# HI-ComputerVision/uni-encoder-code

Measured on AMD Instinct MI355X. Metric: img/s fwd+bwd Swin-L 1024x2048 bs=2 per GPU, higher is better.
Workload: dtype bf16; 1 GPU; BASELINE configs[2]: full OneFormer (Swin-L ws12 backbone + MSDeformAttn pixel decoder + 150-query masked-attention decoder), 1024x2048, fwd+bwd, synthetic loss; global_batch=2, parallelism=dp1, mode=eval() (train_mode reported separately with --full)

## Files before the change

include/uenc.h:

```cpp
#ifndef UENC_H
#define UENC_H
#include <stdint.h>

#ifdef __cplusplus
extern "C" {
#endif

#define UENC_F32 0
#define UENC_BF16 1

#ifndef UENC_STREAM_T
#define UENC_STREAM_T void*
#endif
typedef UENC_STREAM_T uenc_stream_t;

#define UENC_EPI_NONE 0
#define UENC_EPI_GELU 1
#define UENC_EPI_RELU 2
#define UENC_EPI_RESIDUAL 3
#define UENC_EPI_MUL_DGELU 4
#define UENC_EPI_MUL_DRELU 5

int uenc_version(void);
const char* uenc_arch(void);

int uenc_cast_f32_bf16(const float* src, void* dst, long n , uenc_stream_t stream);
int uenc_dropout_bf16(const void* in, void* out, long n, unsigned seed, float p, uenc_stream_t stream);
int uenc_cast_transpose_f32_bf16(const float* src , void* dst , int R, int C, uenc_stream_t stream);

int uenc_cast_multi(const void* table, int n, long total_tiles, uenc_stream_t stream);

int uenc_upsample_bilinear(const float* in, float* out, long NC, int Hi, int Wi, int Ho, int Wo, uenc_stream_t stream);

int uenc_attn_mask(const float* logits, uint8_t* mask, long rows, int Hi, int Wi, int Ho, int Wo, uenc_stream_t stream);

int uenc_add_cast_bf16(const float* a, const float* b, void* out, long n, long period, uenc_stream_t stream);
int uenc_msda_prep_fwd(const float* offaw, long ld, const float* ref, int ref_per_image, const int64_t* shapes, float* loc,
                       float* aw, long rows, int Lq, int M, int L, int P, uenc_stream_t stream);
int uenc_msda_prep_bwd(const float* dloc, const float* daw, const float* aw, const int64_t* shapes, void* doffaw, long ld,
                       long rows, int Lq, int M, int L, int P, uenc_stream_t stream);
int uenc_segment_colsum(const void* x16, long ld, int cols, const int64_t* seg_start, int nseg, long rows_per_image, int images,
                        float* out, uenc_stream_t stream);

long uenc_groupnorm_tokens_scratch_bytes(int B, int HW, int C, int G);
int uenc_groupnorm_tokens_fwd(const void* x, int x_dtype, const float* gamma, const float* beta, void* y, int y_dtype,
                              float* stats, void* scratch, const float* add_src, int Hs, int Ws, int H, int W, int B, int HW,
                              int C, int G, float eps, int relu, uenc_stream_t stream);
int uenc_groupnorm_tokens_bwd(const void* dy, int dy_dtype, const void* x, int x_dtype, const float* gamma, const float* beta,
                              const float* stats, void* dx, int dx_dtype, float* dgamma, float* dbeta, void* scratch, int B,
                              int HW, int C, int G, int relu, uenc_stream_t stream);
int uenc_upsample_bilinear_tokens_bwd(const void* dy, int dy_dtype, float* dsrc, int B, int H, int W, int Hs, int Ws, int C,
                                      uenc_stream_t stream);
int uenc_merge_nearest_tokens_fwd(const void* a, int a_dtype, const void* prev, int prev_dtype, void* out, int out_dtype, int B, int H, int W,
                                  int Hs, int Ws, int C, uenc_stream_t stream);
int uenc_merge_nearest_tokens_bwd(const void* dy, int dy_dtype, float* dprev, int B, int H, int W, int Hs, int Ws, int C,
                                  uenc_stream_t stream);
int uenc_im2col3x3(const void* in, void* col, int B, int H, int W, int C, uenc_stream_t stream);
int uenc_col2im3x3(const void* dcol, void* dx, int B, int H, int W, int C, uenc_stream_t stream);
int uenc_im2col3x3_s2(const void* in, void* col, int B, int H, int W, int C, uenc_stream_t stream);
int uenc_col2im3x3_s2(const void* dcol, float* dx, int B, int H, int W, int C, uenc_stream_t stream);

int uenc_gemm_nt(const void* A, int a_dtype, long lda, const void* W, long ldw, void* C, int c_dtype, long ldc,
                 int M, int N, int K, const float* bias, int epilogue, const void* aux, long ldaux,
                 void* aux_out, long ldaux_out, float alpha, int splitk, int accumulate, uenc_stream_t stream);
#define UENC_NT_TILE_256X256 256
#define UENC_NT_TILE_256X192 192
#define UENC_NT_TILE_128X256 128
int uenc_gemm_nt_tile(const void* A, int a_dtype, long lda, const void* W, long ldw, void* C, int c_dtype, long ldc,
                      int M, int N, int K, const float* bias, int epilogue, const void* aux, long ldaux,
                      void* aux_out, long ldaux_out, float alpha, int splitk, int accumulate, int tile, uenc_stream_t stream);
int uenc_gemm_nt_scaled(const void* A, int a_dtype, long lda, const void* W, long ldw, void* C, int c_dtype, long ldc,
                        int M, int N, int K, const float* bias, int epilogue, const void* aux, long ldaux,
                        void* aux_out, long ldaux_out, float alpha, const float* sample_scale, int rows_per_sample, uenc_stream_t stream);
int uenc_gemm_nt_ln(const void* A, int a_dtype, long lda, const void* W, long ldw, void* C, long ldc, int M, int N, int K, const float* bias,
                    const void* residual, long ldres, const float* gamma, const float* beta, float eps, float* y32, void* y16, float* stats,
                    uenc_stream_t stream);
int uenc_gemm_nt_splits(int K, int splitk);
int uenc_gemm_nt_partials(const void* A, int a_dtype, long lda, const void* W, long ldw, float* P, long ldp, long part_stride,
                          int M, int N, int K, float alpha, int splitk, uenc_stream_t stream);

int uenc_gemm_nt_batched(const void* A, int a_dtype, long lda, long bsA, const void* W, long ldw, long bsW, void* C, int c_dtype,
                         long ldc, long bsC, int batch, int M, int N, int K, float alpha, int splitk, int accumulate, uenc_stream_t stream);

int uenc_gemm_tn(const void* dY, int dy_dtype, long ldy, const void* X, int x_dtype, long ldx, float* dW, long ldw,
                 float* db, int M, int N, int K, int splitm, uenc_stream_t stream);
int uenc_gemm_tn_tile(const void* dY, int dy_dtype, long ldy, const void* X, int x_dtype, long ldx, float* dW, long ldw,
                      float* db, int M, int N, int K, int splitm, int tile, uenc_stream_t stream);
int uenc_gemm_tn_scaled(const void* dY, int dy_dtype, long ldy, const void* X, int x_dtype, long ldx, float* dW, long ldw,
                        float* db, int M, int N, int K, int splitm, float alpha, uenc_stream_t stream);

int uenc_gemm_tn_grouped(const void* table, int n, int total_items, int tile, double flops, uenc_stream_t stream);
int uenc_gemm_tn_grouped_small(const void* table, int n, int total_items, double flops, uenc_stream_t stream);

int uenc_layernorm_fwd(const void* x, int x_dtype, const void* res, int res_dtype, float* h_out, const float* gamma,
                       const float* beta, void* y, int y_dtype, float* stats, long M, int C, float eps, void* y16,
                       uenc_stream_t stream);
int uenc_layernorm_bwd(const void* dy, int dy_dtype, const void* h, int h_dtype, const float* stats, const float* gamma,
                       const float* dres, void* dx, int dx_dtype, float* dgamma, float* dbeta, long M, int C, void* dx16,
                       float* part_ws, int defer_param_sums, uenc_stream_t stream);
int uenc_layernorm_bwd_blocks(long M, int C);
int uenc_ln_param_grouped(const void* table, int n, int total_groups, uenc_stream_t stream);
int uenc_patch_merge_ln_fwd(const float* x, const float* gamma, const float* beta, void* y, float* stats, int B, int H, int W,
                            int C, float eps, uenc_stream_t stream);
int uenc_patch_merge_ln_bwd(const void* dy, int dy_dtype, const float* x, const float* stats, const float* gamma, float* dx,
                            float* dgamma, float* dbeta, float* part_ws, int B, int H, int W, int C, int defer_param_sums,
                            uenc_stream_t stream);

int uenc_window_attn_np(int ws);
int uenc_relpos_expand(const float* table , float* bias_q ,
                       float* bias_k , int nH, int ws, uenc_stream_t stream);
int uenc_relpos_expand_grouped(const void* table, int n, int total_blocks, uenc_stream_t stream);
int uenc_window_attn_fwd(const void* qkv, const void* qkv_bias, const float* bias_q, void* out, float* lse, int B, int H, int W,
                         int C, int nH, int ws, int shift, float scale, uenc_stream_t stream);
long uenc_window_attn_bwd_ws_floats(int B, int H, int W, int nH, int ws);
int uenc_window_attn_bwd(const void* qkv, const void* qkv_bias, const float* bias_q, const float* bias_k,
                         const void* o_saved, const float* lse , const void* d_out, void* dqkv,
                         float* dS_ws, float* dtable, float* dbias_pad,
                         int B, int H, int W, int C, int nH, int ws, int shift, float scale, int defer_dtable, uenc_stream_t stream);
int uenc_window_attn_bwd_groups(int B, int H, int W, int nH, int ws);
int uenc_window_attn_dtable_grouped(const void* table, int n, int total_blocks, uenc_stream_t stream);

int uenc_msdeform_attn_fwd(const void* value, int v_dtype, const int64_t* shapes, const int64_t* level_start,
                           const float* loc, const float* attn, void* out, int out_dtype, int B, int S, int M, int D,
                           int L, int Lq, int P, uenc_stream_t stream);
int uenc_msdeform_attn_fwd_tiled(const void* value, int v_dtype, const int64_t* shapes, const int64_t* level_start,
                                 const float* loc, const float* attn, void* out, int out_dtype, int B, int S, int M, int D,
                                 int L, int Lq, int P, const int64_t* shapes_host, uenc_stream_t stream);
int uenc_msdeform_attn_bwd(const void* value, int v_dtype, const int64_t* shapes, const int64_t* level_start,
                           const float* loc, const float* attn, const void* grad_out, int go_dtype, float* grad_value,
                           float* grad_loc, float* grad_attn, int B, int S, int M, int D, int L, int Lq, int P,
                           const int64_t* shapes_host, void* workspace, long workspace_bytes, uenc_stream_t stream);
long uenc_msdeform_attn_bwd_workspace_bytes(const int64_t* shapes_host, int B, int M, int D, int L, int Lq, int P);
int uenc_msdeform_attn_fused_fwd(const void* value, int v_dtype, const int64_t* shapes, const int64_t* level_start, const float* offaw,
                                 long ld, const float* ref, int ref_per_image, void* out, int out_dtype, int B, int S, int M, int D,
                                 int L, int Lq, int P, uenc_stream_t stream);
int uenc_msdeform_attn_fused_fwd_tiled(const void* value, int v_dtype, const int64_t* shapes, const int64_t* level_start, const float* offaw,
                                       long ld, const float* ref, int ref_per_image, void* out, int out_dtype, int B, int S, int M, int D,
                                       int L, int Lq, int P, const int64_t* shapes_host, uenc_stream_t stream);
int uenc_msdeform_attn_fused_bwd(const void* value, int v_dtype, const int64_t* shapes, const int64_t* level_start, const float* offaw,
                                 long ld, const float* ref, int ref_per_image, const void* grad_out, int go_dtype, float* grad_value,
                                 void* doffaw, long ld_doffaw, int B, int S, int M, int D, int L, int Lq, int P, const int64_t* shapes_host,
                                 void* workspace, long workspace_bytes, uenc_stream_t stream);

long uenc_mha_fwd_workspace_floats(int B, int H, int Lq, int S);
int uenc_mha_fwd(const void* q, long q_bs, long q_rs, const void* k, long k_bs, long k_rs, const void* v, long v_bs,
                 long v_rs, const unsigned char* mask, long mask_rs, void* out, long o_bs, long o_rs, float* lse,
                 float* workspace, int B, int H, int Lq, int S, float scale, float dropout_p, unsigned seed, uenc_stream_t stream);
int uenc_mha_bwd(const void* q, long q_bs, long q_rs, const void* k, long k_bs, long k_rs, const void* v, long v_bs,
                 long v_rs, const unsigned char* mask, long mask_rs, const void* out, long o_bs, long o_rs,
                 const float* lse, const void* dout, long do_bs, long do_rs, float* dq, long dq_bs, long dq_rs, void* dk,
                 long dk_bs, long dk_rs, void* dv, long dv_bs, long dv_rs, int B, int H, int Lq, int S, float scale,
                 float dropout_p, unsigned seed, uenc_stream_t stream);

int uenc_na2d_fwd(const void* qkv, const float* rpb, void* out, float* lse, int B, int H, int W, int nH, int K, int dilation,
                  float scale, uenc_stream_t stream);
int uenc_na2d_bwd(const void* qkv, const float* rpb, const void* out, const void* dout, const float* lse, void* dqkv, float* drpb,
                  float* delta_ws, int B, int H, int W, int nH, int K, int dilation, float scale, uenc_stream_t stream);

int uenc_postproc_semantic(const float* mask_logits, const float* class_prob, float* sem, int Q, int C, int Cp, int hl, int wl,
                           int Hp, int Wp, int Ho, int Wo, uenc_stream_t stream);
int uenc_postproc_panoptic_stats(const float* mask_logits, const float* score, int* ids, int* counts, int Q, int hl, int wl, int Hp,
                                 int Wp, int Ho, int Wo, uenc_stream_t stream);
int uenc_postproc_panoptic_label(const float* mask_logits, const int* ids, const int* segid, int* seg, int Q, int hl, int wl, int Hp,
                                 int Wp, int Ho, int Wo, uenc_stream_t stream);

int uenc_gemm_nt_f32(const float* A, long lda, const float* W, long ldw, float* C, long ldc, int M, int N, int K, const float* bias,
                     int epilogue, const float* aux, long ldaux, float* aux_out, long ldaux_out, float alpha, int accumulate, uenc_stream_t stream);
int uenc_gemm_tn_f32(const float* dY, long ldy, const float* X, long ldx, float* dW, long ldw, float* db, int M, int N, int K, uenc_stream_t stream);
int uenc_window_attn_f32_fwd(const float* qkv, const float* qkv_bias, const float* table, float* out, int B, int H, int W, int C, int nH,
                             int ws, int shift, float scale, uenc_stream_t stream);
int uenc_window_attn_f32_bwd(const float* qkv, const float* qkv_bias, const float* table, const float* dout, float* dqkv, float* dtable,
                             float* dbias_pad, int B, int H, int W, int C, int nH, int ws, int shift, float scale, uenc_stream_t stream);
int uenc_mha_f32_fwd(const float* q, long qs0, long qs1, const float* k, long ks0, long ks1, const float* v, long vs0, long vs1,
                     const uint8_t* mask, long mask_row_stride, float* out, long os0, long os1, float* lse, int B, int nH, int Lq, int S,
                     float scale, float dropout_p, unsigned seed, uenc_stream_t stream);
int uenc_mha_f32_bwd(const float* q, long qs0, long qs1, const float* k, long ks0, long ks1, const float* v, long vs0, long vs1,
                     const uint8_t* mask, long mask_row_stride, const float* out, long os0, long os1, const float* lse, const float* dout,
                     long gos0, long gos1, float* dq, long dqs0, long dqs1, float* dk, long dks0, long dks1, float* dv, long dvs0, long dvs1,
                     float* delta, int B, int nH, int Lq, int S, float scale, float dropout_p, unsigned seed, uenc_stream_t stream);
int uenc_na2d_f32_fwd(const float* qkv, const float* rpb, float* out, float* lse, int B, int H, int W, int nH, int K, int dilation,
                      float scale, uenc_stream_t stream);
int uenc_na2d_f32_bwd(const float* qkv, const float* rpb, const float* out, const float* dout, const float* lse, float* dqkv, float* drpb,
                      int B, int H, int W, int nH, int K, int dilation, float scale, uenc_stream_t stream);
// ... 104 lines not shown
```

uni-encoder-code_amd/csrc/layernorm.hip:

```cpp
#include "common.h"
#include <stdlib.h>

struct LnFwd {
    const void* x; int x_f32;
    const void* res; int res_f32;
    float* h_out;
    const float* gamma; const float* beta;
    void* y; int y_f32;
    bf16* y16;
    float2* stats;
    long M; int C; float eps;
    int mgH, mgW, mgC;
};

struct PatchGather {
    long base; bool ok[4];
    __device__ __forceinline__ PatchGather(long row, int H, int W, int C) {
        const int W2 = (W + 1) >> 1, H2 = (H + 1) >> 1;
        const int j = (int)(row % W2);
        const long r2 = row / W2;
        const int i = (int)(r2 % H2);
        const long b = r2 / H2;
        base = ((b * H + 2 * i) * W + 2 * j) * C;
        const bool y1 = 2 * i + 1 < H, x1 = 2 * j + 1 < W;
        ok[0] = true; ok[1] = y1; ok[2] = x1; ok[3] = y1 && x1;
    }
};
__device__ __forceinline__ void patch_col(int c, int W, int C, int& seg, long& off) {
    seg = c / C;
    off = ((long)(seg & 1) * W + (seg >> 1)) * C + (c - seg * C);
}

__device__ __forceinline__ float4 load4(const void* base, int is_f32, long idx) {
    if (is_f32) return *(const float4*)((const float*)base + idx);
    const bf16x4 v = *(const bf16x4*)((const bf16*)base + idx);
    return make_float4((float)v[0], (float)v[1], (float)v[2], (float)v[3]);
}
__device__ __forceinline__ void store4(void* base, int is_f32, long idx, float4 v) {
    if (is_f32) { *(float4*)((float*)base + idx) = v; return; }
    bf16x4 o; o[0] = (bf16)v.x; o[1] = (bf16)v.y; o[2] = (bf16)v.z; o[3] = (bf16)v.w;
    *(bf16x4*)((bf16*)base + idx) = o;
}

template <int NV, bool MG>
__global__ __launch_bounds__(256) void ln_fwd_kernel(LnFwd p) {
    const int lane = threadIdx.x & 63;
    const long wave0 = (long)blockIdx.x * 4 + (threadIdx.x >> 6);
    const long nwaves = (long)gridDim.x * 4;
    const float invC = 1.0f / (float)p.C;
    int gseg[NV];
    long goff[NV];
    if (MG) {
#pragma unroll
        for (int i = 0; i < NV; ++i) patch_col(min(lane * 4 + i * 256, p.C - 4), p.mgW, p.mgC, gseg[i], goff[i]);
    }
    for (long row = wave0; row < p.M; row += nwaves) {
        float4 v[NV];
        float s = 0.f;
        const PatchGather pg(MG ? row : 0, MG ? p.mgH : 1, MG ? p.mgW : 1, p.mgC);
#pragma unroll
        for (int i = 0; i < NV; ++i) {
            const int c = lane * 4 + i * 256;
            if (c < p.C) {
                if (MG) v[i] = pg.ok[gseg[i]] ? *(const float4*)((const float*)p.x + pg.base + goff[i]) : make_float4(0.f, 0.f, 0.f, 0.f);
                else v[i] = load4(p.x, p.x_f32, row * p.C + c);
                if (p.res != nullptr) {
                    const float4 r = load4(p.res, p.res_f32, row * p.C + c);
                    v[i].x += r.x; v[i].y += r.y; v[i].z += r.z; v[i].w += r.w;
                }
                if (p.h_out != nullptr) *(float4*)(p.h_out + row * p.C + c) = v[i];
                s += v[i].x + v[i].y + v[i].z + v[i].w;
            } else {
                v[i] = make_float4(0.f, 0.f, 0.f, 0.f);
            }
        }
        const float mean = wave_sum(s) * invC;
        float q = 0.f;
#pragma unroll
        for (int i = 0; i < NV; ++i) {
            const int c = lane * 4 + i * 256;
            if (c < p.C) {
                const float a = v[i].x - mean, b = v[i].y - mean, cc = v[i].z - mean, d = v[i].w - mean;
                q += a * a + b * b + cc * cc + d * d;
            }
        }
        const float rstd = rsqrtf(wave_sum(q) * invC + p.eps);
        if (p.stats != nullptr && lane == 0) p.stats[row] = make_float2(mean, rstd);
#pragma unroll
        for (int i = 0; i < NV; ++i) {
            const int c = lane * 4 + i * 256;
            if (c < p.C) {
                const float4 g = *(const float4*)(p.gamma + c), b = *(const float4*)(p.beta + c);
                float4 o;
                o.x = (v[i].x - mean) * rstd * g.x + b.x;
                o.y = (v[i].y - mean) * rstd * g.y + b.y;
                o.z = (v[i].z - mean) * rstd * g.z + b.z;
                o.w = (v[i].w - mean) * rstd * g.w + b.w;
                store4(p.y, p.y_f32, row * p.C + c, o);
                if (p.y16 != nullptr) store4(p.y16, 0, row * p.C + c, o);
            }
        }
    }
}

#define LN_LAUNCH(DIR, NVV, GRID, BLOCK, SHM, STREAM, P)                                                          \
    do {                                                                                                          \
        if ((P).mgC > 0) hipLaunchKernelGGL((ln_##DIR##_kernel<NVV, true>), GRID, BLOCK, SHM, STREAM, P);        \
        else hipLaunchKernelGGL((ln_##DIR##_kernel<NVV, false>), GRID, BLOCK, SHM, STREAM, P);                   \
    } while (0)

static int ln_fwd_launch(LnFwd& p, hipStream_t stream);

extern "C" int uenc_layernorm_fwd(const void* x, int x_dtype, const void* res, int res_dtype, float* h_out,
                                  const float* gamma, const float* beta, void* y, int y_dtype, float* stats,
                                  long M, int C, float eps, void* y16, hipStream_t stream) {
    UENC_CHECK_ARG(x && gamma && beta && y && M > 0 && C > 0 && C % 4 == 0 && C <= 6144);
    LnFwd p;
    p.x = x; p.x_f32 = (x_dtype == UENC_F32); p.res = res; p.res_f32 = (res_dtype == UENC_F32);
    p.h_out = h_out; p.gamma = gamma; p.beta = beta; p.y = y; p.y_f32 = (y_dtype == UENC_F32); p.y16 = (bf16*)y16;
    p.stats = (float2*)stats; p.M = M; p.C = C; p.eps = eps; p.mgH = p.mgW = p.mgC = 0;
    return ln_fwd_launch(p, stream);
}

static int ln_fwd_launch(LnFwd& p, hipStream_t stream) {
// ... 50 lines not shown
        const float2 st = p.stats[row];
        float4 d[NV], xh[NV], rs[NV];
        float s1 = 0.f, s2 = 0.f;
        const PatchGather pg(MG ? row : 0, MG ? p.mgH : 1, MG ? p.mgW : 1, p.mgC);
        if (p.dres != nullptr) {
#pragma unroll
            for (int i = 0; i < NV; ++i) {
                const int c = lane * 4 + i * 256;
                if (c < p.C) rs[i] = *(const float4*)(p.dres + row * p.C + c);
            }
        }
#pragma unroll
        for (int i = 0; i < NV; ++i) {
            const int c = lane * 4 + i * 256;
            if (c < p.C) {
                d[i] = load4(p.dy, p.dy_f32, row * p.C + c);
                float4 hv;
                if (MG) hv = pg.ok[gseg[i]] ? *(const float4*)((const float*)p.h + pg.base + goff[i]) : make_float4(0.f, 0.f, 0.f, 0.f);
                else hv = load4(p.h, p.h_f32, row * p.C + c);
                xh[i] = make_float4((hv.x - st.x) * st.y, (hv.y - st.x) * st.y, (hv.z - st.x) * st.y, (hv.w - st.x) * st.y);
                ag[i].x += d[i].x * xh[i].x; ag[i].y += d[i].y * xh[i].y; ag[i].z += d[i].z * xh[i].z; ag[i].w += d[i].w * xh[i].w;
                ab[i].x += d[i].x; ab[i].y += d[i].y; ab[i].z += d[i].z; ab[i].w += d[i].w;
                d[i].x *= gm[i].x; d[i].y *= gm[i].y; d[i].z *= gm[i].z; d[i].w *= gm[i].w;
                s1 += d[i].x + d[i].y + d[i].z + d[i].w;
                s2 += d[i].x * xh[i].x + d[i].y * xh[i].y + d[i].z * xh[i].z + d[i].w * xh[i].w;
            }
        }
        s1 = wave_sum(s1) * invC;
        s2 = wave_sum(s2) * invC;
#pragma unroll
        for (int i = 0; i < NV; ++i) {
            const int c = lane * 4 + i * 256;
            if (c < p.C) {
                float4 o;
                o.x = st.y * (d[i].x - s1 - xh[i].x * s2);
                o.y = st.y * (d[i].y - s1 - xh[i].y * s2);
                o.z = st.y * (d[i].z - s1 - xh[i].z * s2);
                o.w = st.y * (d[i].w - s1 - xh[i].w * s2);
                if (p.dres != nullptr) { o.x += rs[i].x; o.y += rs[i].y; o.z += rs[i].z; o.w += rs[i].w; }
                if (MG) {
                    if (pg.ok[gseg[i]]) *(float4*)((float*)p.dx + pg.base + goff[i]) = o;
                } else {
                    store4(p.dx, p.dx_f32, row * p.C + c, o);
                    if (p.dx16 != nullptr) store4(p.dx16, 0, row * p.C + c, o);
                }
            }
        }
    }
    if (p.dgamma != nullptr && p.C > 2048) {
        for (int c = threadIdx.x; c < 2 * p.C; c += 256) sh[c] = 0.f;
        __syncthreads();
#pragma unroll
        for (int i = 0; i < NV; ++i) {
            const int c = lane * 4 + i * 256;
            if (c < p.C) {
                atomicAdd(&sh[c + 0], ag[i].x); atomicAdd(&sh[c + 1], ag[i].y);
                atomicAdd(&sh[c + 2], ag[i].z); atomicAdd(&sh[c + 3], ag[i].w);
                atomicAdd(&sh[p.C + c + 0], ab[i].x); atomicAdd(&sh[p.C + c + 1], ab[i].y);
                atomicAdd(&sh[p.C + c + 2], ab[i].z); atomicAdd(&sh[p.C + c + 3], ab[i].w);
            }
        }
        __syncthreads();
        for (int c = threadIdx.x; c < 2 * p.C; c += 256) {
            if (p.part != nullptr) p.part[(long)blockIdx.x * 2 * p.C + c] = sh[c];
            else atomicAdd((c < p.C ? p.dgamma + c : p.dbeta + (c - p.C)), sh[c]);
        }
    } else if (p.dgamma != nullptr) {
        const int wv = threadIdx.x >> 6;
        float* mine = sh + (long)wv * 2 * p.C;
#pragma unroll
        for (int i = 0; i < NV; ++i) {
            const int c = lane * 4 + i * 256;
            if (c < p.C) { *(float4*)(mine + c) = ag[i]; *(float4*)(mine + p.C + c) = ab[i]; }
        }
        __syncthreads();
        for (int c = threadIdx.x; c < 2 * p.C; c += 256) {
            const float v = sh[c] + sh[2 * p.C + c] + sh[4 * p.C + c] + sh[6 * p.C + c];
            if (p.part != nullptr) p.part[(long)blockIdx.x * 2 * p.C + c] = v;
            else atomicAdd((c < p.C ? p.dgamma + c : p.dbeta + (c - p.C)), v);
        }
    }
}

__global__ __launch_bounds__(256) void ln_bwd_param_kernel(const float* __restrict__ part, int nblk, int C, float* __restrict__ dgamma,
                                                           float* __restrict__ dbeta) {
    __shared__ float red[4][64];
    const int col = blockIdx.x * 64 + (threadIdx.x & 63), r = threadIdx.x >> 6;
    const int per = (nblk + gridDim.y - 1) / gridDim.y, b0 = blockIdx.y * per, b1 = min(nblk, b0 + per);
    float acc = 0.f;
    if (col < 2 * C)
        for (int b = b0 + r; b < b1; b += 4) acc += part[(long)b * 2 * C + col];
    red[r][threadIdx.x & 63] = acc;
    __syncthreads();
    if (r == 0 && col < 2 * C) {
        const float v = red[0][threadIdx.x] + red[1][threadIdx.x] + red[2][threadIdx.x] + red[3][threadIdx.x];
        atomicAdd(col < C ? dgamma + col : dbeta + (col - C), v);
    }
}

static int ln_bwd_launch(LnBwd& p, float* part_ws, int defer, hipStream_t stream);

extern "C" int uenc_layernorm_bwd(const void* dy, int dy_dtype, const void* h, int h_dtype, const float* stats,
                                  const float* gamma, const float* dres, void* dx, int dx_dtype, float* dgamma,
                                  float* dbeta, long M, int C, void* dx16, float* part_ws, int defer_param_sums, hipStream_t stream) {
    UENC_CHECK_ARG(dy && h && stats && gamma && dx && M > 0 && C > 0 && C % 4 == 0 && C <= 6144);
    UENC_CHECK_ARG((dgamma == nullptr) == (dbeta == nullptr));
    LnBwd p;
    p.dy = dy; p.dy_f32 = (dy_dtype == UENC_F32); p.h = h; p.h_f32 = (h_dtype == UENC_F32);
    p.stats = (const float2*)stats; p.gamma = gamma; p.dres = dres; p.dx = dx; p.dx_f32 = (dx_dtype == UENC_F32); p.dx16 = (bf16*)dx16;
    p.dgamma = dgamma; p.dbeta = dbeta; p.M = M; p.C = C; p.mgH = p.mgW = p.mgC = 0;
    return ln_bwd_launch(p, part_ws, defer_param_sums, stream);
}

static long ln_bwd_blocks(long M, int C, bool with_ws, bool* stored) {
    long blocks = (M + 3) / 4;
    long cap = with_ws ? 2048 : 1024;
    { const char* e = getenv("UENC_LN_BWD_BLOCKS"); if (e && atoi(e) >= 64 && atoi(e) <= 2048) cap = atoi(e); }
    if (blocks > cap) blocks = cap;
    *stored = with_ws && blocks * 2 * C > 131072;
    return blocks;
}

extern "C" int uenc_layernorm_bwd_blocks(long M, int C) {
    if (M <= 0 || C <= 0) return 0;
    bool stored = false;
    const long b = ln_bwd_blocks(M, C, true, &stored);
    return stored ? (int)b : 0;
}

static int ln_bwd_launch(LnBwd& p, float* part_ws, int defer, hipStream_t stream) {
    const long M = p.M; const int C = p.C;
    float* dgamma = p.dgamma; float* dbeta = p.dbeta;
    bool stored = false;
    const long blocks = ln_bwd_blocks(M, C, part_ws != nullptr && dgamma != nullptr, &stored);
    p.part = stored ? part_ws : nullptr;
    const int nv = (C + 255) / 256;
    const size_t shm = (size_t)(C > 2048 ? 1 : 4) * 2 * C * sizeof(float);
    dim3 grid((unsigned)blocks), block(256);
    if (nv <= 1) LN_LAUNCH(bwd, 1, grid, block, shm, stream, p);
    else if (nv <= 2) LN_LAUNCH(bwd, 2, grid, block, shm, stream, p);
    else if (nv <= 4) LN_LAUNCH(bwd, 4, grid, block, shm, stream, p);
    else if (nv <= 8) LN_LAUNCH(bwd, 8, grid, block, shm, stream, p);
    else if (nv <= 16) LN_LAUNCH(bwd, 16, grid, block, shm, stream, p);
    else LN_LAUNCH(bwd, 24, grid, block, shm, stream, p);
    if (p.part != nullptr && !defer)
        hipLaunchKernelGGL(ln_bwd_param_kernel, dim3((2 * C + 63) / 64, 16), dim3(256), 0, stream, (const float*)p.part, (int)blocks, C, dgamma, dbeta);
    UENC_LAUNCH_RET();
}

struct LnParamDesc { const float* part; float* dgamma; float* dbeta; int nblk, C, group_begin, pad; };
__global__ __launch_bounds__(256) void ln_param_grouped_kernel(const LnParamDesc* __restrict__ table, int n) {
    __shared__ float red[4][64];
    int lo = 0, hi = n - 1;
    const int grp = blockIdx.x;
    while (lo < hi) {
        const int mid = (lo + hi + 1) >> 1;
        if (table[mid].group_begin <= grp) lo = mid; else hi = mid - 1;
    }
    const LnParamDesc d = table[lo];
    const int C = d.C, nblk = d.nblk;
    const int col = (grp - d.group_begin) * 64 + (threadIdx.x & 63), r = threadIdx.x >> 6;
    const int per = (nblk + gridDim.y - 1) / gridDim.y, b0 = blockIdx.y * per, b1 = min(nblk, b0 + per);
    float acc = 0.f;
    if (col < 2 * C)
        for (int b = b0 + r; b < b1; b += 4) acc += d.part[(long)b * 2 * C + col];
    red[r][threadIdx.x & 63] = acc;
    __syncthreads();
    if (r == 0 && col < 2 * C) {
        const float v = red[0][threadIdx.x] + red[1][threadIdx.x] + red[2][threadIdx.x] + red[3][threadIdx.x];
        atomicAdd(col < C ? d.dgamma + col : d.dbeta + (col - C), v);
    }
}

extern "C" int uenc_ln_param_grouped(const void* table, int n, int total_groups, hipStream_t stream) {
    UENC_CHECK_ARG(table && n > 0 && total_groups > 0 && ((uintptr_t)table & 7) == 0);
    static_assert(sizeof(LnParamDesc) == 40, "descriptor layout is part of the ABI");
    hipLaunchKernelGGL(ln_param_grouped_kernel, dim3((unsigned)total_groups, 16), dim3(256), 0, stream, (const LnParamDesc*)table, n);
    UENC_LAUNCH_RET();
}


extern "C" int uenc_patch_merge_ln_fwd(const float* x, const float* gamma, const float* beta, void* y, float* stats, int B, int H, int W,
                                       int C, float eps, hipStream_t stream) {
    UENC_CHECK_ARG(x && gamma && beta && y && stats && B > 0 && H > 0 && W > 0 && C > 0 && C % 4 == 0 && 4 * C <= 6144);
    UENC_CHECK_ARG((((uintptr_t)x | (uintptr_t)y) & 15) == 0);
    LnFwd p;
    p.x = x; p.x_f32 = 1; p.res = nullptr; p.res_f32 = 0; p.h_out = nullptr; p.gamma = gamma; p.beta = beta; p.y = y; p.y_f32 = 0;
    p.y16 = nullptr; p.stats = (float2*)stats; p.M = (long)B * ((H + 1) / 2) * ((W + 1) / 2); p.C = 4 * C; p.eps = eps;
    p.mgH = H; p.mgW = W; p.mgC = C;
    return ln_fwd_launch(p, stream);
}

extern "C" int uenc_patch_merge_ln_bwd(const void* dy, int dy_dtype, const float* x, const float* stats, const float* gamma, float* dx,
                                       float* dgamma, float* dbeta, float* part_ws, int B, int H, int W, int C, int defer_param_sums,
                                       hipStream_t stream) {
    UENC_CHECK_ARG(dy && x && stats && gamma && dx && B > 0 && H > 0 && W > 0 && C > 0 && C % 4 == 0 && 4 * C <= 6144);
    UENC_CHECK_ARG((dgamma == nullptr) == (dbeta == nullptr));
    LnBwd p;
    p.dy = dy; p.dy_f32 = (dy_dtype == UENC_F32); p.h = x; p.h_f32 = 1; p.stats = (const float2*)stats; p.gamma = gamma; p.dres = nullptr;
    p.dx = dx; p.dx_f32 = 1; p.dx16 = nullptr; p.dgamma = dgamma; p.dbeta = dbeta;
    p.M = (long)B * ((H + 1) / 2) * ((W + 1) / 2); p.C = 4 * C; p.mgH = H; p.mgW = W; p.mgC = C;
    return ln_bwd_launch(p, part_ws, defer_param_sums, stream);
}
```

uni-encoder-code_amd/uenc/capi.py:

```python
import ctypes
import os

import torch

_HERE = os.path.dirname(os.path.abspath(__file__))
LIB_PATH = os.path.join(_HERE, "libuenc_hip.so")

F32, BF16 = 0, 1
EPI_NONE, EPI_GELU, EPI_RELU, EPI_RESIDUAL, EPI_MUL_DGELU, EPI_MUL_DRELU = range(6)

c_p, c_i, c_l, c_f, c_u, c_d = ctypes.c_void_p, ctypes.c_int, ctypes.c_long, ctypes.c_float, ctypes.c_uint, ctypes.c_double

_SIGNATURES = {
    "uenc_version": [],
    "uenc_prof_enable": [c_i],
    "uenc_prof_collect": [c_i, c_p, c_p, c_p],
    "uenc_prof_collect_bytes": [c_i, c_p],
    "uenc_prof_next_bytes": [ctypes.c_double],
    "uenc_cast_f32_bf16": [c_p, c_p, c_l, c_p],
    "uenc_cast_transpose_f32_bf16": [c_p, c_p, c_i, c_i, c_p],
    "uenc_cast_multi": [c_p, c_i, c_l, c_p],
    "uenc_upsample_bilinear": [c_p, c_p, c_l, c_i, c_i, c_i, c_i, c_p],
    "uenc_attn_mask": [c_p, c_p, c_l, c_i, c_i, c_i, c_i, c_p],
    "uenc_gemm_nt": [c_p, c_i, c_l, c_p, c_l, c_p, c_i, c_l, c_i, c_i, c_i, c_p, c_i, c_p, c_l, c_p, c_l, c_f, c_i, c_i, c_p],
    "uenc_gemm_nt_tile": [c_p, c_i, c_l, c_p, c_l, c_p, c_i, c_l, c_i, c_i, c_i, c_p, c_i, c_p, c_l, c_p, c_l, c_f, c_i, c_i, c_i, c_p],
    "uenc_gemm_nt_scaled": [c_p, c_i, c_l, c_p, c_l, c_p, c_i, c_l, c_i, c_i, c_i, c_p, c_i, c_p, c_l, c_p, c_l, c_f, c_p, c_i, c_p],
    "uenc_gemm_nt_ln": [c_p, c_i, c_l, c_p, c_l, c_p, c_l, c_i, c_i, c_i, c_p, c_p, c_l, c_p, c_p, c_f, c_p, c_p, c_p, c_p],
    "uenc_groupnorm_tokens_scratch_bytes": [c_i, c_i, c_i, c_i],
    "uenc_groupnorm_tokens_fwd": [c_p, c_i, c_p, c_p, c_p, c_i, c_p, c_p, c_p, c_i, c_i, c_i, c_i, c_i, c_i, c_i, c_i, c_f, c_i, c_p],
    "uenc_groupnorm_tokens_bwd": [c_p, c_i, c_p, c_i, c_p, c_p, c_p, c_p, c_i, c_p, c_p, c_p, c_i, c_i, c_i, c_i, c_i, c_p],
    "uenc_upsample_bilinear_tokens_bwd": [c_p, c_i, c_p, c_i, c_i, c_i, c_i, c_i, c_i, c_p],
    "uenc_merge_nearest_tokens_fwd": [c_p, c_i, c_p, c_i, c_p, c_i, c_i, c_i, c_i, c_i, c_i, c_i, c_p],
    "uenc_merge_nearest_tokens_bwd": [c_p, c_i, c_p, c_i, c_i, c_i, c_i, c_i, c_i, c_p],
    "uenc_im2col3x3": [c_p, c_p, c_i, c_i, c_i, c_i, c_p],
    "uenc_col2im3x3": [c_p, c_p, c_i, c_i, c_i, c_i, c_p],
    "uenc_add_cast_bf16": [c_p, c_p, c_p, c_l, c_l, c_p],
    "uenc_msda_prep_fwd": [c_p, c_l, c_p, c_i, c_p, c_p, c_p, c_l, c_i, c_i, c_i, c_i, c_p],
    "uenc_msda_prep_bwd": [c_p, c_p, c_p, c_p, c_p, c_l, c_l, c_i, c_i, c_i, c_i, c_p],
    "uenc_segment_colsum": [c_p, c_l, c_i, c_p, c_i, c_l, c_i, c_p, c_p],
    "uenc_dropout_bf16": [c_p, c_p, c_l, c_u, c_f, c_p],
    "uenc_gemm_nt_splits": [c_i, c_i],
    "uenc_gemm_nt_partials": [c_p, c_i, c_l, c_p, c_l, c_p, c_l, c_l, c_i, c_i, c_i, c_f, c_i, c_p],
    "uenc_gemm_nt_batched": [c_p, c_i, c_l, c_l, c_p, c_l, c_l, c_p, c_i, c_l, c_l, c_i, c_i, c_i, c_i, c_f, c_i, c_i, c_p],
    "uenc_gemm_tn": [c_p, c_i, c_l, c_p, c_i, c_l, c_p, c_l, c_p, c_i, c_i, c_i, c_i, c_p],
    "uenc_gemm_tn_tile": [c_p, c_i, c_l, c_p, c_i, c_l, c_p, c_l, c_p, c_i, c_i, c_i, c_i, c_i, c_p],
    "uenc_gemm_tn_scaled": [c_p, c_i, c_l, c_p, c_i, c_l, c_p, c_l, c_p, c_i, c_i, c_i, c_i, c_f, c_p],
    "uenc_gemm_tn_grouped": [c_p, c_i, c_i, c_i, ctypes.c_double, c_p],
    "uenc_gemm_tn_grouped_small": [c_p, c_i, c_i, ctypes.c_double, c_p],
    "uenc_layernorm_fwd": [c_p, c_i, c_p, c_i, c_p, c_p, c_p, c_p, c_i, c_p, c_l, c_i, c_f, c_p, c_p],
    "uenc_layernorm_bwd": [c_p, c_i, c_p, c_i, c_p, c_p, c_p, c_p, c_i, c_p, c_p, c_l, c_i, c_p, c_p, c_i, c_p],
    "uenc_layernorm_bwd_blocks": [c_l, c_i],
    "uenc_ln_param_grouped": [c_p, c_i, c_i, c_p],
    "uenc_window_attn_bwd_groups": [c_i, c_i, c_i, c_i, c_i],
    "uenc_window_attn_dtable_grouped": [c_p, c_i, c_i, c_p],
    "uenc_msdeform_attn_fwd": [c_p, c_i, c_p, c_p, c_p, c_p, c_p, c_i, c_i, c_i, c_i, c_i, c_i, c_i, c_i, c_p],
    "uenc_msdeform_attn_fwd_tiled": [c_p, c_i, c_p, c_p, c_p, c_p, c_p, c_i, c_i, c_i, c_i, c_i, c_i, c_i, c_i, c_p, c_p],
    "uenc_msdeform_attn_bwd": [c_p, c_i, c_p, c_p, c_p, c_p, c_p, c_i, c_p, c_p, c_p, c_i, c_i, c_i, c_i, c_i, c_i, c_i, c_p, c_p, c_l, c_p],
    "uenc_msdeform_attn_bwd_workspace_bytes": [c_p, c_i, c_i, c_i, c_i, c_i, c_i],
    "uenc_msdeform_attn_fused_fwd": [c_p, c_i, c_p, c_p, c_p, c_l, c_p, c_i, c_p, c_i, c_i, c_i, c_i, c_i, c_i, c_i, c_i, c_p],
    "uenc_msdeform_attn_fused_fwd_tiled": [c_p, c_i, c_p, c_p, c_p, c_l, c_p, c_i, c_p, c_i, c_i, c_i, c_i, c_i, c_i, c_i, c_i, c_p, c_p],
    "uenc_msdeform_attn_fused_bwd": [c_p, c_i, c_p, c_p, c_p, c_l, c_p, c_i, c_p, c_i, c_p, c_p, c_l, c_i, c_i, c_i, c_i, c_i, c_i, c_i, c_p, c_p, c_l, c_p],
    "uenc_mha_fwd_workspace_floats": [c_i, c_i, c_i, c_i],
    "uenc_mha_fwd": [c_p, c_l, c_l, c_p, c_l, c_l, c_p, c_l, c_l, c_p, c_l, c_p, c_l, c_l, c_p, c_p, c_i, c_i, c_i, c_i, c_f, c_f, c_u, c_p],
    "uenc_mha_bwd": [c_p, c_l, c_l, c_p, c_l, c_l, c_p, c_l, c_l, c_p, c_l, c_p, c_l, c_l, c_p, c_p, c_l, c_l, c_p, c_l, c_l,
                     c_p, c_l, c_l, c_p, c_l, c_l, c_i, c_i, c_i, c_i, c_f, c_f, c_u, c_p],
    "uenc_window_attn_np": [c_i],
    "uenc_relpos_expand": [c_p, c_p, c_p, c_i, c_i, c_p],
    "uenc_relpos_expand_grouped": [c_p, c_i, c_i, c_p],
    "uenc_window_attn_fwd": [c_p, c_p, c_p, c_p, c_p, c_i, c_i, c_i, c_i, c_i, c_i, c_i, c_f, c_p],
    "uenc_postproc_semantic": [c_p, c_p, c_p, c_i, c_i, c_i, c_i, c_i, c_i, c_i, c_i, c_i, c_p],
    "uenc_postproc_panoptic_stats": [c_p, c_p, c_p, c_p, c_i, c_i, c_i, c_i, c_i, c_i, c_i, c_p],
    "uenc_postproc_panoptic_label": [c_p, c_p, c_p, c_p, c_i, c_i, c_i, c_i, c_i, c_i, c_i, c_p],
    "uenc_patch_merge_ln_fwd": [c_p, c_p, c_p, c_p, c_p, c_i, c_i, c_i, c_i, c_f, c_p],
    "uenc_patch_merge_ln_bwd": [c_p, c_i, c_p, c_p, c_p, c_p, c_p, c_p, c_p, c_i, c_i, c_i, c_i, c_i, c_p],
    "uenc_im2col3x3_s2": [c_p, c_p, c_i, c_i, c_i, c_i, c_p],
    "uenc_col2im3x3_s2": [c_p, c_p, c_i, c_i, c_i, c_i, c_p],
    "uenc_na2d_fwd": [c_p, c_p, c_p, c_p, c_i, c_i, c_i, c_i, c_i, c_i, c_f, c_p],
    "uenc_na2d_bwd": [c_p, c_p, c_p, c_p, c_p, c_p, c_p, c_p, c_i, c_i, c_i, c_i, c_i, c_i, c_f, c_p],
    "uenc_window_attn_bwd_ws_floats": [c_i, c_i, c_i, c_i, c_i],
    "uenc_step_rng_advance": [c_p, c_p, c_i, c_i, c_p, c_i, c_p, c_i, c_p],
    "uenc_dropout_sp": [c_p, c_p, c_l, c_i, c_p, c_i, c_f, c_p],
    "uenc_upload": [c_p, c_p, c_l, c_p],
    "uenc_prof_active": [],
    "uenc_scale_rows_bf16": [c_p, c_l, c_p, c_l, c_l, c_i, c_p, c_l, c_p],
    "uenc_mha_fwd_sp": [c_p, c_l, c_l, c_p, c_l, c_l, c_p, c_l, c_l, c_p, c_l, c_p, c_l, c_l, c_p, c_p, c_i, c_i, c_i, c_i, c_f, c_f, c_p, c_i, c_p],
    "uenc_mha_bwd_sp": [c_p, c_l, c_l, c_p, c_l, c_l, c_p, c_l, c_l, c_p, c_l, c_p, c_l, c_l, c_p, c_p, c_l, c_l, c_p, c_l, c_l,
                        c_p, c_l, c_l, c_p, c_l, c_l, c_i, c_i, c_i, c_i, c_f, c_f, c_p, c_i, c_p],
    "uenc_attn_tiled_tile": [c_i],
    "uenc_attn_tiled_fwd": [c_p, c_l, c_l, c_p, c_l, c_l, c_p, c_l, c_l, c_p, c_l, c_l, c_p, c_i, c_i, c_i, c_i, c_f, c_f, c_u, c_p],
    "uenc_attn_tiled_bwd": [c_p, c_l, c_l, c_p, c_l, c_l, c_p, c_l, c_l, c_p, c_l, c_l, c_p, c_p, c_l, c_l, c_p, c_l, c_l,
                            c_p, c_l, c_l, c_p, c_l, c_l, c_i, c_i, c_i, c_i, c_f, c_f, c_u, c_p],
    "uenc_attn_tiled_fwd_sp": [c_p, c_l, c_l, c_p, c_l, c_l, c_p, c_l, c_l, c_p, c_l, c_l, c_p, c_i, c_i, c_i, c_i, c_f, c_f, c_p, c_i, c_p],
    "uenc_attn_tiled_bwd_sp": [c_p, c_l, c_l, c_p, c_l, c_l, c_p, c_l, c_l, c_p, c_l, c_l, c_p, c_p, c_l, c_l, c_p, c_l, c_l,
                               c_p, c_l, c_l, c_p, c_l, c_l, c_i, c_i, c_i, c_i, c_f, c_f, c_p, c_i, c_p],
    "uenc_gemm_nt_f32": [c_p, c_l, c_p, c_l, c_p, c_l, c_i, c_i, c_i, c_p, c_i, c_p, c_l, c_p, c_l, c_f, c_i, c_p],
    "uenc_gemm_tn_f32": [c_p, c_l, c_p, c_l, c_p, c_l, c_p, c_i, c_i, c_i, c_p],
    "uenc_window_attn_f32_fwd": [c_p, c_p, c_p, c_p, c_i, c_i, c_i, c_i, c_i, c_i, c_i, c_f, c_p],
    "uenc_window_attn_f32_bwd": [c_p, c_p, c_p, c_p, c_p, c_p, c_p, c_i, c_i, c_i, c_i, c_i, c_i, c_i, c_f, c_p],
    "uenc_mha_f32_fwd": [c_p, c_l, c_l, c_p, c_l, c_l, c_p, c_l, c_l, c_p, c_l, c_p, c_l, c_l, c_p, c_i, c_i, c_i, c_i, c_f, c_f, c_u, c_p],
    "uenc_mha_f32_bwd": [c_p, c_l, c_l, c_p, c_l, c_l, c_p, c_l, c_l, c_p, c_l, c_p, c_l, c_l, c_p, c_p, c_l, c_l, c_p, c_l, c_l,
                         c_p, c_l, c_l, c_p, c_l, c_l, c_p, c_i, c_i, c_i, c_i, c_f, c_f, c_u, c_p],
    "uenc_na2d_f32_fwd": [c_p, c_p, c_p, c_p, c_i, c_i, c_i, c_i, c_i, c_i, c_f, c_p],
    "uenc_na2d_f32_bwd": [c_p, c_p, c_p, c_p, c_p, c_p, c_p, c_i, c_i, c_i, c_i, c_i, c_i, c_f, c_p],
    "uenc_window_attn_bwd": [c_p, c_p, c_p, c_p, c_p, c_p, c_p, c_p, c_p, c_p, c_p, c_i, c_i, c_i, c_i, c_i, c_i, c_i, c_f, c_i, c_p],
    "uenc_optim_advance": [c_p, c_d, c_d, c_p],
    "uenc_optim_grad_sqnorm": [c_p, c_i, c_l, c_p, c_i, c_p, c_f, c_p],
    "uenc_optim_adamw_step": [c_p, c_i, c_l, c_p, c_i, c_p, c_d, c_d, c_d, c_p],
    "uenc_match_cost_workspace_floats": [c_i, c_i, c_i, c_i],
    "uenc_match_cost": [c_p, c_i, c_i, c_i, c_i, c_i, c_i, c_i, c_i, c_i, c_f, c_f, c_f, c_f, c_p, c_l, c_p, c_p],
    "uenc_lsap_solve": [c_p, c_i, c_i, c_p],
    "uenc_crit_point_logits": [c_p, c_i, c_i, c_i, c_i, c_i, c_i, c_i, c_p, c_p, c_p, c_p],
    "uenc_crit_mask_loss_fwd": [c_p, c_i, c_i, c_i, c_i, c_i, c_i, c_i, c_i, c_i, c_p, c_p, c_p, c_p, c_p, c_p, c_p, c_p],
    "uenc_crit_mask_loss_bwd": [c_p, c_i, c_i, c_i, c_i, c_i, c_i, c_i, c_p, c_p, c_p, c_p, c_p, c_p, c_p, c_f, c_p, c_p],
    "uenc_crit_class_loss": [c_p, c_i, c_i, c_i, c_i, c_i, c_p, c_p, c_f, c_p, c_p, c_p, c_p],
    "uenc_view_synth_workspace_floats": [c_i, c_i, c_i, c_i, c_i],
    "uenc_view_synth_fwd": [c_p, c_i, c_i, c_i, c_i, c_i, c_i, c_p],
    "uenc_view_synth_bwd": [c_p, c_i, c_i, c_i, c_i, c_i, c_i, c_p, c_l, c_p],
    "uenc_photo_loss_workspace_floats": [c_i, c_i, c_i, c_i],
    "uenc_photo_loss_fwd": [c_p, c_p, c_p, c_p, c_i, c_i, c_i, c_i, c_i, c_i, c_p, c_l, c_p, c_p, c_p],
    "uenc_photo_loss_bwd": [c_p, c_p, c_p, c_p, c_i, c_i, c_i, c_i, c_i, c_i, c_p, c_p],
    "uenc_dwconv7_ln_fwd": [c_p, c_p, c_p, c_p, c_p, c_p, c_p, c_i, c_p, c_i, c_i, c_i, c_i, c_f, c_p],
    "uenc_dwconv7_ln_bwd_data": [c_p, c_i, c_p, c_p, c_p, c_p, c_p, c_p, c_p, c_p, c_p, c_p, c_i, c_i, c_i, c_i, c_i, c_p],
    "uenc_dwconv7_bwd_weight_workspace_bytes": [c_i, c_i, c_i, c_i],
    "uenc_dwconv7_bwd_weight": [c_p, c_p, c_p, c_p, c_p, c_l, c_i, c_i, c_i, c_i, c_p],
    "uenc_layer_scale_grads": [c_p, c_p, c_p, c_p, c_p, c_p, c_p, c_p, c_i, c_i, c_p],
    "uenc_stem7x7_s2_patches": [c_p, c_p, c_i, c_i, c_i, c_i, c_p],
    "uenc_maxpool3x3_s2_fwd": [c_p, c_p, c_p, c_i, c_i, c_i, c_i, c_i, c_p],
    "uenc_maxpool3x3_s2_bwd": [c_p, c_p, c_p, c_i, c_i, c_i, c_i, c_i, c_p],
    "uenc_bn_workspace_floats": [c_l, c_i],
    "uenc_bn_stats": [c_p, c_i, c_l, c_i, c_p, c_p, c_p, c_p, c_p, c_f, c_p, c_l, c_p],
    "uenc_bn_act_fwd": [c_p, c_i, c_p, c_p, c_p, c_p, c_p, c_i, c_p, c_i, c_l, c_i, c_f, c_i, c_p],
    "uenc_bn_act_bwd_reduce": [c_p, c_i, c_p, c_i, c_p, c_i, c_p, c_p, c_l, c_i, c_f, c_i, c_p, c_p, c_p, c_p, c_l, c_p],
    "uenc_bn_act_bwd_apply": [c_p, c_i, c_p, c_i, c_p, c_i, c_p, c_p, c_p, c_p, c_p, c_i, c_p, c_i, c_l, c_i, c_f, c_i, c_i, c_p],
}


class UencError(RuntimeError):
    pass


def _load():
    if not os.path.exists(LIB_PATH):
        raise ImportError(
            f"{LIB_PATH} is missing: build it with `python -c 'import __graft_entry__ as g; g.build()'` "
            "(or `make -C uni-encoder-code_amd/csrc`). The HIP library is mandatory; there is no fallback path.")
    lib = ctypes.CDLL(LIB_PATH)
    for name, argtypes in _SIGNATURES.items():
        fn = getattr(lib, name)
        fn.argtypes = argtypes
        fn.restype = c_i
    lib.uenc_window_attn_bwd_ws_floats.restype = c_l
    lib.uenc_mha_fwd_workspace_floats.restype = c_l
    lib.uenc_msdeform_attn_bwd_workspace_bytes.restype = c_l
    lib.uenc_groupnorm_tokens_scratch_bytes.restype = c_l
    lib.uenc_match_cost_workspace_floats.restype = c_l
    lib.uenc_view_synth_workspace_floats.restype = c_l
    lib.uenc_photo_loss_workspace_floats.restype = c_l
    lib.uenc_dwconv7_bwd_weight_workspace_bytes.restype = c_l
    lib.uenc_bn_workspace_floats.restype = c_l
    lib.uenc_arch.restype = ctypes.c_char_p
    lib.uenc_arch.argtypes = []
    return lib


lib = _load()


def exported_symbols():
    return sorted(list(_SIGNATURES) + ["uenc_arch"])


def check(code: int, what: str = "uenc"):
    if code == 0:
        return
    if code < 0:
        raise UencError(f"{what}: invalid argument (shape / alignment / dtype), nothing was launched")
    raise UencError(f"{what}: hipError_t {code}")


def stream_ptr():
    return torch.cuda.current_stream().cuda_stream


def dt(t: torch.Tensor) -> int:
    if t.dtype == torch.float32:
        return F32
    if t.dtype == torch.bfloat16:
        return BF16
    raise UencError(f"unsupported dtype {t.dtype}")


def ptr(t):
    return 0 if t is None else t.data_ptr()
```

Before: 30.98 img/s.

## Split LayerNorm backward rows across multiple waves with prefetch and LDS reduction

Adds a LayerNorm backward kernel that spreads one row over several waves (WPR) and packs several rows per workgroup when C is small. Row reductions are combined across waves through a double-buffered LDS array plus a DPP wave sum, and the next row's raw loads are prefetched to overlap memory latency. The aim is better occupancy and latency hiding than the old one-wave-per-row kernel, which held many float4 values per lane for wide C. The cost is a __syncthreads per row and more LDS. A helper exposing the row stride is also exported.

```diff
diff --git a/include/uenc.h b/include/uenc.h
--- a/include/uenc.h
+++ b/include/uenc.h
@@ -99,6 +99,7 @@
                        const float* dres, void* dx, int dx_dtype, float* dgamma, float* dbeta, long M, int C, void* dx16,
                        float* part_ws, int defer_param_sums, uenc_stream_t stream);
 int uenc_layernorm_bwd_blocks(long M, int C);
+long uenc_layernorm_bwd_row_stride(long M, int C, int param_grads);
 int uenc_ln_param_grouped(const void* table, int n, int total_groups, uenc_stream_t stream);
 int uenc_patch_merge_ln_fwd(const float* x, const float* gamma, const float* beta, void* y, float* stats, int B, int H, int W,
                             int C, float eps, uenc_stream_t stream);
diff --git a/uni-encoder-code_amd/csrc/layernorm.hip b/uni-encoder-code_amd/csrc/layernorm.hip
--- a/uni-encoder-code_amd/csrc/layernorm.hip
+++ b/uni-encoder-code_amd/csrc/layernorm.hip
@@ -15,6 +15,8 @@
 
 struct PatchGather {
     long base; bool ok[4];
+    unsigned mask;
+    __device__ __forceinline__ bool has(int seg) const { return (mask >> seg) & 1u; }
     __device__ __forceinline__ PatchGather(long row, int H, int W, int C) {
         const int W2 = (W + 1) >> 1, H2 = (H + 1) >> 1;
         const int j = (int)(row % W2);
@@ -24,6 +26,7 @@
         base = ((b * H + 2 * i) * W + 2 * j) * C;
         const bool y1 = 2 * i + 1 < H, x1 = 2 * j + 1 < W;
         ok[0] = true; ok[1] = y1; ok[2] = x1; ok[3] = y1 && x1;
+        mask = 1u | (y1 ? 2u : 0u) | (x1 ? 4u : 0u) | (y1 && x1 ? 8u : 0u);
     }
 };
 __device__ __forceinline__ void patch_col(int c, int W, int C, int& seg, long& off) {
@@ -40,6 +43,30 @@
     if (is_f32) { *(float4*)((float*)base + idx) = v; return; }
     bf16x4 o; o[0] = (bf16)v.x; o[1] = (bf16)v.y; o[2] = (bf16)v.z; o[3] = (bf16)v.w;
     *(bf16x4*)((bf16*)base + idx) = o;
+}
+
+__device__ __forceinline__ u32x4 load_raw4(const void* base, int is_f32, long idx) {
+    if (is_f32) return *(const u32x4*)((const float*)base + idx);
+    const u32x2 v = *(const u32x2*)((const bf16*)base + idx);
+    u32x4 r = {v[0], v[1], 0u, 0u};
+    return r;
+}
+__device__ __forceinline__ float4 widen4(u32x4 r, int is_f32) {
+    if (is_f32) return make_float4(__uint_as_float(r[0]), __uint_as_float(r[1]), __uint_as_float(r[2]), __uint_as_float(r[3]));
+    u32x2 u = {r[0], r[1]};
+    const bf16x4 v = __builtin_bit_cast(bf16x4, u);
+    return make_float4((float)v[0], (float)v[1], (float)v[2], (float)v[3]);
+}
+
+__device__ __forceinline__ float wave_sum_valu(float v) {
+    v = xor32_sum(v);
+    v = xor16_sum(v);
+    v = dpp_add_f32<0x128>(v);
+    int t = __builtin_amdgcn_update_dpp(0, __builtin_bit_cast(int, v), 0x104, 0xf, 0x5, false);
+    t = __builtin_amdgcn_update_dpp(t, __builtin_bit_cast(int, v), 0x114, 0xf, 0xa, false);
+    v += __builtin_bit_cast(float, t);
+    v = dpp_add_f32<0x4E>(v);
+    return dpp_add_f32<0xB1>(v);
 }
 
 template <int NV, bool MG>
@@ -256,6 +283,133 @@
     }
 }
 
+template <int NV, int WPR, int NW, bool MG>
+__global__ __launch_bounds__(NW * 64) void ln_bwd_split_kernel(LnBwd p) {
+    constexpr int RPW = NW / WPR, NK = NV * WPR;
+    __shared__ float T[2][RPW][2][NK][64];
+    extern __shared__ __attribute__((aligned(16))) float sh[];
+    const int lane = threadIdx.x & 63, wv = threadIdx.x >> 6, grp = wv / WPR, wr = wv % WPR;
+    const float invC = 1.0f / (float)p.C;
+    int col[NV], gseg[NV];
+    long goff[NV];
+    bool in[NV];
+    float4 ag[NV], ab[NV], gm[NV];
+#pragma unroll
+    for (int i = 0; i < NV; ++i) {
+        col[i] = (i * WPR + wr) * 256 + lane * 4;
+        in[i] = col[i] < p.C;
+        ag[i] = make_float4(0.f, 0.f, 0.f, 0.f);
+        ab[i] = ag[i];
+        gm[i] = in[i] ? *(const float4*)(p.gamma + col[i]) : ag[i];
+        gseg[i] = 0; goff[i] = 0;
+        if (MG) patch_col(min(col[i], p.C - 4), p.mgW, p.mgC, gseg[i], goff[i]);
+    }
+    const long stride = (long)gridDim.x * RPW;
+    const long iters = (p.M + stride - 1) / stride;
+    struct Row { u32x4 dy[NV], h[NV]; float4 rs[NV]; float2 st; long base; unsigned ok; };
+    auto fetch = [&](long row, Row& r) {
+        const PatchGather pg(MG ? row : 0, MG ? p.mgH : 1, MG ? p.mgW : 1, p.mgC);
+        r.base = pg.base; r.ok = pg.mask;
+        if (row >= p.M) return;
+        r.st = p.stats[row];
+#pragma unroll
+        for (int i = 0; i < NV; ++i) {
+            if (!in[i]) continue;
+            if (p.dres != nullptr) r.rs[i] = *(const float4*)(p.dres + row * p.C + col[i]);
+            r.dy[i] = load_raw4(p.dy, p.dy_f32, row * p.C + col[i]);
+            if (MG) {
+                const u32x4 z = {0u, 0u, 0u, 0u};
+                r.h[i] = pg.has(gseg[i]) ? *(const u32x4*)((const float*)p.h + pg.base + goff[i]) : z;
+            } else {
+                r.h[i] = load_raw4(p.h, p.h_f32, row * p.C + col[i]);
+            }
+        }
+    };
+    long row = (long)blockIdx.x * RPW + grp;
+    Row cur;
+    fetch(row, cur);
+    for (long it = 0; it < iters; ++it, row += stride) {
+        Row nxt;
+        fetch(row + stride, nxt);
+        const bool valid = row < p.M;
+        const float2 st = cur.st;
+        float4 d[NV], xh[NV];
+        float (*Tb)[NK][64] = T[it & 1][grp];
+#pragma unroll
+        for (int i = 0; i < NV; ++i) {
+            float t1 = 0.f, t2 = 0.f;
+            if (valid && in[i]) {
+                d[i] = widen4(cur.dy[i], p.dy_f32);
+                const float4 hv = widen4(cur.h[i], MG ? 1 : p.h_f32);
+                xh[i] = make_float4((hv.x - st.x) * st.y, (hv.y - st.x) * st.y, (hv.z - st.x) * st.y, (hv.w - st.x) * st.y);
+                ag[i].x += d[i].x * xh[i].x; ag[i].y += d[i].y * xh[i].y; ag[i].z += d[i].z * xh[i].z; ag[i].w += d[i].w * xh[i].w;
+                ab[i].x += d[i].x; ab[i].y += d[i].y; ab[i].z += d[i].z; ab[i].w += d[i].w;
+                d[i].x *= gm[i].x; d[i].y *= gm[i].y; d[i].z *= gm[i].z; d[i].w *= gm[i].w;
+                t1 = d[i].x + d[i].y + d[i].z + d[i].w;
+                t2 = d[i].x * xh[i].x + d[i].y * xh[i].y + d[i].z * xh[i].z + d[i].w * xh[i].w;
+            }
+            Tb[0][i * WPR + wr][lane] = t1;
+            Tb[1][i * WPR + wr][lane] = t2;
+        }
+        __syncthreads();
+        float s1 = 0.f, s2 = 0.f;
+#pragma unroll
+        for (int k = 0; k < NK; ++k) {
+            if (k * 256 + lane * 4 < p.C) { s1 += Tb[0][k][lane]; s2 += Tb[1][k][lane]; }
+        }
+        s1 = wave_sum_valu(s1) * invC;
+        s2 = wave_sum_valu(s2) * invC;
+#pragma unroll
+        for (int i = 0; i < NV; ++i) {
+            if (valid && in[i]) {
+                float4 o;
+                o.x = st.y * (d[i].x - s1 - xh[i].x * s2);
+                o.y = st.y * (d[i].y - s1 - xh[i].y * s2);
+                o.z = st.y * (d[i].z - s1 - xh[i].z * s2);
+                o.w = st.y * (d[i].w - s1 - xh[i].w * s2);
+                if (p.dres != nullptr) { o.x += cur.rs[i].x; o.y += cur.rs[i].y; o.z += cur.rs[i].z; o.w += cur.rs[i].w; }
+                if (MG) {
+                    if ((cur.ok >> gseg[i]) & 1u) *(float4*)((float*)p.dx + cur.base + goff[i]) = o;
+                } else {
+                    store4(p.dx, p.dx_f32, row * p.C + col[i], o);
+                    if (p.dx16 != nullptr) store4(p.dx16, 0, row * p.C + col[i], o);
+                }
+            }
+        }
+        cur = nxt;
+    }
+    if (p.dgamma == nullptr) return;
+    if (RPW == 1) {
+#pragma unroll
+        for (int i = 0; i < NV; ++i) {
+            if (!in[i]) continue;
+            if (p.part != nullptr) {
+                float* mine = p.part + (long)blockIdx.x * 2 * p.C + col[i];
+                *(float4*)mine = ag[i];
+                *(float4*)(mine + p.C) = ab[i];
+            } else {
+                float* g = p.dgamma + col[i]; float* b = p.dbeta + col[i];
+                atomicAdd(g + 0, ag[i].x); atomicAdd(g + 1, ag[i].y); atomicAdd(g + 2, ag[i].z); atomicAdd(g + 3, ag[i].w);
+                atomicAdd(b + 0, ab[i].x); atomicAdd(b + 1, ab[i].y); atomicAdd(b + 2, ab[i].z); atomicAdd(b + 3, ab[i].w);
+            }
+        }
+    } else {
+        float* mine = sh + (long)grp * 2 * p.C;
+#pragma unroll
+        for (int i = 0; i < NV; ++i) {
+            if (in[i]) { *(float4*)(mine + col[i]) = ag[i]; *(float4*)(mine + p.C + col[i]) = ab[i]; }
+        }
+        __syncthreads();
+        for (int c = threadIdx.x; c < 2 * p.C; c += NW * 64) {
+            float v = sh[c];
+#pragma unroll
+            for (int g = 1; g < RPW; ++g) v += sh[g * 2 * p.C + c];
+            if (p.part != nullptr) p.part[(long)blockIdx.x * 2 * p.C + c] = v;
+            else atomicAdd((c < p.C ? p.dgamma + c : p.dbeta + (c - p.C)), v);
+        }
+    }
+}
+
 __global__ __launch_bounds__(256) void ln_bwd_param_kernel(const float* __restrict__ part, int nblk, int C, float* __restrict__ dgamma,
                                                            float* __restrict__ dbeta) {
     __shared__ float red[4][64];
@@ -302,21 +456,35 @@
     return stored ? (int)b : 0;
 }
 
+#define LN_SPLIT_DISPATCH(NVC, F, ...)                                                                             \
+    ((NVC) <= 2 ? F<1, 2, 4>(__VA_ARGS__) : (NVC) == 3 ? F<1, 3, 3>(__VA_ARGS__) : (NVC) <= 4 ? F<1, 4, 4>(__VA_ARGS__) \
+     : (NVC) <= 8 ? F<1, 8, 8>(__VA_ARGS__) : (NVC) <= 16 ? F<1, 16, 16>(__VA_ARGS__) : F<2, 16, 16>(__VA_ARGS__))
+static int ln_bwd_rows_per_workgroup(int nvc) { return nvc <= 1 ? 4 : nvc <= 2 ? 2 : 1; }
+
+template <int NV, int WPR, int NW>
+static int ln_bwd_split_launch(const LnBwd& p, long blocks, hipStream_t stream) {
+    constexpr int RPW = NW / WPR;
+    const size_t shm = RPW > 1 ? (size_t)RPW * 2 * p.C * sizeof(float) : 0;
+    if (p.mgC > 0) hipLaunchKernelGGL((ln_bwd_split_kernel<NV, WPR, NW, true>), dim3((unsigned)blocks), dim3(NW * 64), shm, stream, p);
+    else hipLaunchKernelGGL((ln_bwd_split_kernel<NV, WPR, NW, false>), dim3((unsigned)blocks), dim3(NW * 64), shm, stream, p);
+    return 0;
+}
+
+extern "C" long uenc_layernorm_bwd_row_stride(long M, int C, int param_grads) {
+    if (M <= 0 || C <= 0 || C % 4 != 0 || C > 6144) return 0;
+    bool stored = false;
+    return ln_bwd_blocks(M, C, param_grads != 0, &stored) * ln_bwd_rows_per_workgroup((C + 255) / 256);
+}
+
 static int ln_bwd_launch(LnBwd& p, float* part_ws, int defer, hipStream_t stream) {
     const long M = p.M; const int C = p.C;
     float* dgamma = p.dgamma; float* dbeta = p.dbeta;
     bool stored = false;
     const long blocks = ln_bwd_blocks(M, C, part_ws != nullptr && dgamma != nullptr, &stored);
     p.part = stored ? part_ws : nullptr;
-    const int nv = (C + 255) / 256;
-    const size_t shm = (size_t)(C > 2048 ? 1 : 4) * 2 * C * sizeof(float);
-    dim3 grid((unsigned)blocks), block(256);
-    if (nv <= 1) LN_LAUNCH(bwd, 1, grid, block, shm, stream, p);
-    else if (nv <= 2) LN_LAUNCH(bwd, 2, grid, block, shm, stream, p);
-    else if (nv <= 4) LN_LAUNCH(bwd, 4, grid, block, shm, stream, p);
-    else if (nv <= 8) LN_LAUNCH(bwd, 8, grid, block, shm, stream, p);
-    else if (nv <= 16) LN_LAUNCH(bwd, 16, grid, block, shm, stream, p);
-    else LN_LAUNCH(bwd, 24, grid, block, shm, stream, p);
+    const int nvc = (C + 255) / 256;
+    if (nvc <= 1) LN_LAUNCH(bwd, 1, dim3((unsigned)blocks), dim3(256), (size_t)4 * 2 * C * sizeof(float), stream, p);
+    else (void)LN_SPLIT_DISPATCH(nvc, ln_bwd_split_launch, p, blocks, stream);
     if (p.part != nullptr && !defer)
         hipLaunchKernelGGL(ln_bwd_param_kernel, dim3((2 * C + 63) / 64, 16), dim3(256), 0, stream, (const float*)p.part, (int)blocks, C, dgamma, dbeta);
     UENC_LAUNCH_RET();
diff --git a/uni-encoder-code_amd/uenc/capi.py b/uni-encoder-code_amd/uenc/capi.py
--- a/uni-encoder-code_amd/uenc/capi.py
+++ b/uni-encoder-code_amd/uenc/capi.py
@@ -50,6 +50,7 @@
     "uenc_layernorm_fwd": [c_p, c_i, c_p, c_i, c_p, c_p, c_p, c_p, c_i, c_p, c_l, c_i, c_f, c_p, c_p],
     "uenc_layernorm_bwd": [c_p, c_i, c_p, c_i, c_p, c_p, c_p, c_p, c_i, c_p, c_p, c_l, c_i, c_p, c_p, c_i, c_p],
     "uenc_layernorm_bwd_blocks": [c_l, c_i],
+    "uenc_layernorm_bwd_row_stride": [c_l, c_i, c_i],
     "uenc_ln_param_grouped": [c_p, c_i, c_i, c_p],
     "uenc_window_attn_bwd_groups": [c_i, c_i, c_i, c_i, c_i],
     "uenc_window_attn_dtable_grouped": [c_p, c_i, c_i, c_p],
@@ -158,6 +159,7 @@
     lib.uenc_photo_loss_workspace_floats.restype = c_l
     lib.uenc_dwconv7_bwd_weight_workspace_bytes.restype = c_l
     lib.uenc_bn_workspace_floats.restype = c_l
+    lib.uenc_layernorm_bwd_row_stride.restype = c_l
     lib.uenc_arch.restype = ctypes.c_char_p
     lib.uenc_arch.argtypes = []
     return lib
```

Measured after the change: 31.25 img/s (median of 3 runs). About the same (+0.9%).
